# NilFoundation/crypto3-zk

Hardware: AMD Instinct MI355X
Metric: MSM Mpoints/sec, BLS12-381 G1 Pippenger, 2^20 points per GPU (higher is better)
Workload: dtype u32; 1 GPU; BLS12-381 G1 Pippenger MSM, ONE MSM of 1 x 2^20 random points/scalars, bases resident; points_per_gpu=1048576, parallelism=point-range partition x1 + one all-gather of the 144-B partial sums

## Files before the change

__graft_entry__.py:

```python
import importlib.util
import os
import subprocess
import sys

ROOT = os.path.dirname(os.path.abspath(__file__))


def _load_pkg():
    if "crypto3_zk_amd" in sys.modules:
        return sys.modules["crypto3_zk_amd"]
    pkg_dir = os.path.join(ROOT, "crypto3-zk_amd")
    spec = importlib.util.spec_from_file_location("crypto3_zk_amd", os.path.join(pkg_dir, "__init__.py"),
                                                  submodule_search_locations=[pkg_dir])
    mod = importlib.util.module_from_spec(spec)
    sys.modules["crypto3_zk_amd"] = mod
    spec.loader.exec_module(mod)
    return mod


def build() -> None:
    env = dict(os.environ)
    subprocess.check_call(["make", "-C", os.path.join(ROOT, "crypto3-zk_amd"), "-j4", "all"], env=env)
    subprocess.check_call(["make", "-C", os.path.join(ROOT, "oracle"), "liboracle.so"], env=env)
    subprocess.check_call(["make", "-j2", "-C", os.path.join(ROOT, "tests", "cpp")], env=env)
    subprocess.check_call(["make", "-C", os.path.join(ROOT, "tests", "cpp"), "-f", "merkle.mk"], env=env)
    subprocess.check_call(["make", "-C", os.path.join(ROOT, "tests", "cpp"), "-f", "pow.mk"], env=env)
    subprocess.check_call(["make", "-j2", "-C", os.path.join(ROOT, "tests", "cpp"), "-f", "pasta.mk"], env=env)
    subprocess.check_call(["make", "-C", os.path.join(ROOT, "tests", "cpp"), "-f", "wide.mk"], env=env)
    subprocess.check_call(["make", "-C", os.path.join(ROOT, "tests", "cpp"), "-f", "entries.mk"], env=env)
    subprocess.check_call(["make", "-C", os.path.join(ROOT, "tests", "cpp"), "-f", "ipa.mk"], env=env)
    subprocess.check_call(["make", "-C", os.path.join(ROOT, "tests", "cpp"), "-f", "lagrange.mk"], env=env)
    subprocess.check_call(["make", "-C", os.path.join(ROOT, "tests", "cpp"), "-f", "ceremony.mk"], env=env)
    subprocess.check_call(["make", "-C", os.path.join(ROOT, "tests", "cpp"), "-f", "fri_query.mk"], env=env)
    subprocess.check_call(["make", "-C", os.path.join(ROOT, "tests", "cpp"), "-f", "ipp2.mk"], env=env)
    zk = _load_pkg()
    zk.load_library()


def smoke() -> None:
    import numpy as np

    sys.path.insert(0, os.path.join(ROOT, "oracle"))
    import cport as cp
    import pyoracle as po

    zk = _load_pkg()
    ctx = zk.Context(0)
    n = 5000
    ks = cp.random_fr(0, 1, n)
    bases = ctx.bases_from_scalars(zk.BLS12_381, zk.G1, ks)
    pts, inf = bases.download()
    exp_pts, _ = cp.batch_mul(0, 1, ks)
    assert (pts == exp_pts).all(), "device fixed-base multiples differ from the oracle"
    sc = cp.random_fr(0, 2, n)
    aff, is_inf = ctx.msm_affine(bases, sc)
    exp, einf = cp.msm(0, 1, pts, sc, chunks=2)
    assert is_inf == einf and (aff == exp).all(), "MSM differs from the oracle"
    grp = zk.DeviceGroup([0, 0])
    gb = grp.upload_bases(zk.BLS12_381, zk.G1, pts)
    gaff, ginf = grp.msm_affine(gb, sc)
    assert ginf == einf and (gaff == exp).all(), "device-group MSM differs from the oracle"
    gb.free()
    grp.close()
    k2 = cp.random_fr(0, 4, 300)
    b2 = ctx.bases_from_scalars(zk.BLS12_381, zk.G2, k2)
    p2, _ = b2.download()
    s2 = cp.random_fr(0, 5, 300)
    aff2, inf2 = ctx.msm_affine(b2, s2)
    exp2, einf2 = cp.msm(0, 2, p2, s2, chunks=2)
    assert inf2 == einf2 and (aff2 == exp2).all(), "G2 MSM differs from the oracle"
    b2.free()
    log_m = 12
    w = np.array(po.to_limbs(po.BLS12_381.root_of_unity(log_m), 4), dtype=np.uint64)
    a = cp.random_fr(0, 3, 2 << log_m).reshape(2, 1 << log_m, 4)
    got = ctx.ntt(zk.BLS12_381, a, log_m, w)
    assert (got == cp.ntt(0, a, log_m, w)).all(), "NTT differs from the oracle"
    assert (ctx.ntt(zk.BLS12_381, got, log_m, w, inverse=True) == a).all()
    bases.free()
    M, nin = 1024, 10
    g16 = cp.Groth16(0, M, nin, seed=3)
    kind, m = cp.domain_choice(M + nin + 1, 32)
    wd = np.array(po.to_limbs(po.BLS12_381.root_of_unity((M + nin).bit_length()), 4), dtype=np.uint64)
    gen = np.array(po.to_limbs(po.BLS12_381.fr_generator, 4), dtype=np.uint64)
    g16.set_domain(kind, m, wd)
    r1cs = ctx.upload_r1cs(zk.BLS12_381, g16.M, g16.n, g16.N, g16.csr(0), g16.csr(1), g16.csr(2))
    assert (r1cs.kind, r1cs.m) == (kind, m) == (2, 1040), "the constraint system's domain is not the reference's choice"
    z = np.concatenate([np.array([[1, 0, 0, 0]], dtype=np.uint64), g16.assignment()])
    assert (ctx.groth16_witness_h(r1cs, z, wd, gen) == g16.witness_map(wd, gen)).all(), "witness map over the step domain differs from the oracle"
    r1cs.free()
    import hashlib
    state = hashlib.sha256(b"zkhip smoke").digest()
    k = next(k for k in range(1 << 20)
             if int.from_bytes(hashlib.sha256(hashlib.sha256(state + (12345 + k).to_bytes(4, "big")).digest()).digest()[28:], "big") & 0xFFF == 0)
    assert ctx.pow_grind(state, 12345, 0xFFF) == (12345 + k, k + 1), "the device's proof of work is not the first accepted nonce"
    ctx.close()
    print("smoke ok: G1 MSM n=5000 (one context and a device group of two), G2 MSM n=300, NTT 2^12 x 2 and the witness map over a step radix-2 domain bit-exact against the oracle; proof of work (12 bits) = the reference loop's nonce")


if __name__ == "__main__":
    build()
    if len(sys.argv) > 1 and sys.argv[1] == "smoke":
        smoke()
```

crypto3-zk_amd/csrc/msm_entries.hip:

```cpp
#include <algorithm>
#include <string>

#include "ctx.hpp"
#include "fu.hpp"
#include "msm_entries.hpp"
#include "msm_ops.hpp"
#include "msm_recode.hpp"

namespace {

using namespace zkhip;

constexpr uint32_t MSM_LARGE_BUCKET = 128;
constexpr uint32_t MSM_LARGE_CHUNK = 4096;

template <uint32_t THREADS>
ZK_D void block_inclusive_scan(uint32_t *scratch) {
    const uint32_t t = threadIdx.x;
    __syncthreads();
    for (uint32_t d = 1; d < THREADS; d <<= 1) {
        uint32_t x = t >= d ? scratch[t - d] : 0;
        __syncthreads();
        scratch[t] += x;
        __syncthreads();
    }
}

__global__ __launch_bounds__(256) void msm_scan_local(const uint32_t *__restrict__ hist, uint32_t count, uint32_t *__restrict__ offs,
                                                      uint32_t *__restrict__ block_sums) {
    __shared__ uint32_t part[256];
    const uint32_t t = threadIdx.x, base = blockIdx.x * 1024 + t * 4;
    uint32_t v[4], s = 0;
#pragma unroll
    for (int k = 0; k < 4; ++k) {
        v[k] = base + k < count ? hist[base + k] : 0;
        s += v[k];
    }
    part[t] = s;
    block_inclusive_scan<256>(part);
    uint32_t run = part[t] - s;
#pragma unroll
    for (int k = 0; k < 4; ++k) {
        if (base + k < count) offs[base + k] = run;
        run += v[k];
    }
    if (t == 255) block_sums[blockIdx.x] = part[255];
}

__global__ __launch_bounds__(1024) void msm_scan_top(uint32_t *__restrict__ block_sums, uint32_t nblocks, uint32_t *__restrict__ total) {
    __shared__ uint32_t part[1024];
    const uint32_t t = threadIdx.x;
    const uint32_t per = (nblocks + 1023) / 1024;
    const uint32_t lo = min(nblocks, t * per), hi = min(nblocks, lo + per);
    uint32_t s = 0;
    for (uint32_t i = lo; i < hi; ++i) s += block_sums[i];
    part[t] = s;
    block_inclusive_scan<1024>(part);
    uint32_t run = part[t] - s;
    for (uint32_t i = lo; i < hi; ++i) {
        uint32_t x = block_sums[i];
        block_sums[i] = run;
        run += x;
    }
    if (t == 1023) *total = part[1023];
}

__global__ __launch_bounds__(256) void msm_scan_add(uint32_t *__restrict__ offs, uint32_t count, const uint32_t *__restrict__ block_sums,
                                                    uint32_t *__restrict__ cursor) {
    const uint32_t base = blockIdx.x * 1024 + threadIdx.x * 4;
    const uint32_t add = block_sums[blockIdx.x];
#pragma unroll
    for (int k = 0; k < 4; ++k) {
        if (base + k < count) {
            uint32_t x = offs[base + k] + add;
            offs[base + k] = x;
            cursor[base + k] = x;
        }
    }
}

__global__ __launch_bounds__(1024) void msm_scan_single(const uint32_t *__restrict__ hist, uint32_t count, uint32_t *__restrict__ offs,
                                                        uint32_t *__restrict__ cursor) {
    __shared__ uint32_t part[1024];
    __shared__ uint32_t carry;
    const uint32_t t = threadIdx.x;
    if (t == 0) carry = 0;
    __syncthreads();
    for (uint32_t base = 0; base < count; base += 1024) {
        const uint32_t v = base + t < count ? hist[base + t] : 0;
        part[t] = v;
        block_inclusive_scan<1024>(part);
        const uint32_t excl = carry + part[t] - v;
        if (base + t < count) {
            offs[base + t] = excl;
            if (cursor != offs) cursor[base + t] = excl;
        }
        __syncthreads();
        if (t == 1023) carry += part[1023];
        __syncthreads();
    }
    if (t == 0) offs[count] = carry;
}
constexpr uint32_t MSM_SCAN_SINGLE_MAX = 1u << 16;

inline int msm_scan(zkhip_ctx *ctx, const char *name, const uint32_t *hist, uint32_t count, uint32_t *offs, uint32_t *bsums) {
    if (count <= MSM_SCAN_SINGLE_MAX) {
        ZK_LAUNCH(ctx, name, msm_scan_single, dim3(1), dim3(1024), 0, hist, count, offs, offs);
        return 0;
    }
    const uint32_t nblk = (count + 1023) / 1024;
    ZK_LAUNCH(ctx, name, msm_scan_local, dim3(nblk), dim3(256), 0, hist, count, offs, bsums);
    ZK_LAUNCH(ctx, name, msm_scan_top, dim3(1), dim3(1024), 0, bsums, nblk, offs + count);
    ZK_LAUNCH(ctx, name, msm_scan_add, dim3(nblk), dim3(256), 0, offs, count, bsums, offs);
    return 0;
}

template <class FR>
__global__ __launch_bounds__(256) void msm_digits_only(const uint32_t *__restrict__ scalars, uint32_t n, MsmWindows win, uint32_t wrank,
                                                       uint32_t wworld, uint32_t *__restrict__ dig) {
    uint32_t i = blockIdx.x * blockDim.x + threadIdx.x;
    if (i >= n) return;
    uint32_t s[8];
    const uint32_t flip = msm_fold_scalar<FR>(scalars + (size_t)i * 8, s) ? 0x80000000u : 0u;
    uint32_t carry = 0, next = wrank, lw = 0;
    for (int w = 0; w < win.W; ++w) {
        uint32_t d = msm_recode(s, win.off(w), win.width(w), carry);
        if ((uint32_t)w != next) continue;
        dig[(size_t)lw * n + i] = d == DIG_NONE ? d : d ^ flip;
        next += wworld;
        ++lw;
    }
}

struct SortBig {
    static constexpr uint32_t TILE = 16384, THREADS = 1024;
};
struct SortSmall {
    static constexpr uint32_t TILE = 4096, THREADS = 256;
};
constexpr uint32_t SORT_MAX_LOW = 10;
constexpr uint32_t SORT_MAX_SUPER = 1024;

ZK_D uint32_t sort_key(const SortGeom &g, uint32_t w, uint32_t d) { return (w % g.S) * g.B + (d & 0x7FFFFFFFu); }
ZK_D uint32_t sort_entry(const SortGeom &g, uint32_t w, uint32_t i, uint32_t d) {
    return ((g.tables ? (g.slot0 + w) * g.bases_n : 0u) + g.base_off + i) | (d & 0x80000000u);
}

template <class SZ>
__global__ __launch_bounds__(SZ::THREADS) void msm_sort_hist(const uint32_t *__restrict__ dig, SortGeom g, uint32_t *__restrict__ bh) {
    constexpr uint32_t SORT_TILE = SZ::TILE, SORT_THREADS = SZ::THREADS;
    extern __shared__ uint32_t lh[];
    const uint32_t tile = blockIdx.x, w = blockIdx.y, t = threadIdx.x;
    for (uint32_t k = t; k < g.nsuper; k += SORT_THREADS) lh[k] = 0;
    __syncthreads();
    const uint32_t lo = tile * SORT_TILE, hi = min(g.n, lo + SORT_TILE);
    for (uint32_t i = lo + t; i < hi; i += SORT_THREADS) {
        uint32_t d = dig[(size_t)w * g.n + i];
        if (d != DIG_NONE) atomicAdd(&lh[sort_key(g, w, d) >> g.lowb], 1u);
    }
    __syncthreads();
    const size_t col = (size_t)w * g.ntile + tile, stride = (size_t)g.W * g.ntile;
    for (uint32_t k = t; k < g.nsuper; k += SORT_THREADS) bh[(size_t)k * stride + col] = lh[k];
}

template <uint32_t SORT_THREADS>
ZK_D uint32_t block_excl_scan(uint32_t *v, uint32_t count, uint32_t *scratch ) {
    const uint32_t t = threadIdx.x, per = (count + SORT_THREADS - 1) / SORT_THREADS;
    const uint32_t lo = min(count, t * per), hi = min(count, lo + per);
    uint32_t s = 0;
    for (uint32_t k = lo; k < hi; ++k) s += v[k];
    scratch[t] = s;
    block_inclusive_scan<SORT_THREADS>(scratch);
    const uint32_t total = scratch[SORT_THREADS - 1];
    uint32_t run = scratch[t] - s;
    for (uint32_t k = lo; k < hi; ++k) {
        uint32_t x = v[k];
        v[k] = run;
        run += x;
    }
    __syncthreads();
    return total;
}

template <class SZ>
__global__ __launch_bounds__(SZ::THREADS) void msm_sort_split(const uint32_t *__restrict__ dig, SortGeom g, const uint32_t *__restrict__ bo,
                                                              uint32_t *__restrict__ tmp_idx, uint16_t *__restrict__ tmp_key) {
    constexpr uint32_t SORT_TILE = SZ::TILE, SORT_THREADS = SZ::THREADS;
    extern __shared__ uint32_t sm[];
    uint32_t *loff = sm;
    uint32_t *cur = loff + g.nsuper + 1;
    uint32_t *gbase = cur + g.nsuper;
    uint32_t *scratch = gbase + g.nsuper;
    uint32_t *sidx = scratch + SORT_THREADS;
    uint32_t *skey = sidx + SORT_TILE;
    const uint32_t tile = blockIdx.x, w = blockIdx.y, t = threadIdx.x;
    const size_t col = (size_t)w * g.ntile + tile, stride = (size_t)g.W * g.ntile;
    for (uint32_t k = t; k < g.nsuper; k += SORT_THREADS) {
        loff[k] = 0;
        gbase[k] = bo[(size_t)k * stride + col];
    }
    __syncthreads();
    const uint32_t lo = tile * SORT_TILE, hi = min(g.n, lo + SORT_TILE);
    for (uint32_t i = lo + t; i < hi; i += SORT_THREADS) {
        uint32_t d = dig[(size_t)w * g.n + i];
        if (d != DIG_NONE) atomicAdd(&loff[sort_key(g, w, d) >> g.lowb], 1u);
    }
    __syncthreads();
    const uint32_t total = block_excl_scan<SORT_THREADS>(loff, g.nsuper, scratch);
    if (t == 0) loff[g.nsuper] = total;
    for (uint32_t k = t; k < g.nsuper; k += SORT_THREADS) cur[k] = loff[k];
    __syncthreads();
    for (uint32_t i = lo + t; i < hi; i += SORT_THREADS) {
        uint32_t d = dig[(size_t)w * g.n + i];
        if (d == DIG_NONE) continue;
        const uint32_t key = sort_key(g, w, d);
        const uint32_t r = atomicAdd(&cur[key >> g.lowb], 1u);
        sidx[r] = sort_entry(g, w, i, d);
        skey[r] = key;
    }
    __syncthreads();
    const uint32_t lmask = (1u << g.lowb) - 1;
    for (uint32_t s = t; s < total; s += SORT_THREADS) {
        const uint32_t key = skey[s], bin = key >> g.lowb, pos = gbase[bin] + (s - loff[bin]);
        tmp_idx[pos] = sidx[s];
        tmp_key[pos] = (uint16_t)(key & lmask);
    }
}

constexpr uint32_t SORT_NLOW_MAX = 1u << SORT_MAX_LOW;

template <uint32_t THREADS>
ZK_D void block_scan_counts(const uint32_t *cnt, uint32_t *excl, uint32_t *scratch) {
    constexpr uint32_t CPT = SORT_NLOW_MAX / THREADS;
    const uint32_t t = threadIdx.x;
    uint32_t s = 0;
#pragma unroll
    for (uint32_t k = 0; k < CPT; ++k) s += cnt[t * CPT + k];
    scratch[t] = s;
    block_inclusive_scan<THREADS>(scratch);
    uint32_t run = scratch[t] - s;
#pragma unroll
    for (uint32_t k = 0; k < CPT; ++k) {
        excl[t * CPT + k] = run;
        run += cnt[t * CPT + k];
    }
    __syncthreads();
}

template <class SZ>
__global__ __launch_bounds__(SZ::THREADS) void msm_sort_final(const uint32_t *__restrict__ tmp_idx, const uint16_t *__restrict__ tmp_key, SortGeom g,
                                                              uint32_t nb, const uint32_t *__restrict__ bo, uint32_t *__restrict__ offs,
                                                              uint32_t *__restrict__ idx) {
    constexpr uint32_t SORT_TILE = SZ::TILE, SORT_THREADS = SZ::THREADS;
    __shared__ uint32_t cnt[SORT_NLOW_MAX], cursor[SORT_NLOW_MAX], loff[SORT_NLOW_MAX], cur[SORT_NLOW_MAX], scratch[SORT_THREADS];
    extern __shared__ uint32_t sm[];
    uint32_t *sidx = sm;
    uint16_t *skey = reinterpret_cast<uint16_t *>(sidx + SORT_TILE);
    const uint32_t grp = blockIdx.x, t = threadIdx.x;
    const size_t stride = (size_t)g.W * g.ntile;
    const uint32_t start = bo[(size_t)grp * stride];
    const uint32_t end = bo[(size_t)(grp + 1) * stride];
    const uint32_t nlow = 1u << g.lowb;
    for (uint32_t k = t; k < SORT_NLOW_MAX; k += SORT_THREADS) cnt[k] = 0;
    __syncthreads();
    for (uint32_t k = start + t; k < end; k += SORT_THREADS) atomicAdd(&cnt[tmp_key[k]], 1u);
    __syncthreads();
    block_scan_counts<SORT_THREADS>(cnt, cursor, scratch);
    for (uint32_t k = t; k < nlow; k += SORT_THREADS) {
        const uint32_t bucket = grp * nlow + k;
        cursor[k] += start;
        if (bucket < nb) offs[bucket] = cursor[k];
    }
    if (grp + 1 == g.nsuper && t == 0) offs[nb] = end;
    __syncthreads();
    for (uint32_t c0 = start; c0 < end; c0 += SORT_TILE) {
        const uint32_t c1 = min(end, c0 + SORT_TILE);
        for (uint32_t k = t; k < SORT_NLOW_MAX; k += SORT_THREADS) cnt[k] = 0;
        __syncthreads();
        for (uint32_t k = c0 + t; k < c1; k += SORT_THREADS) atomicAdd(&cnt[tmp_key[k]], 1u);
        __syncthreads();
        block_scan_counts<SORT_THREADS>(cnt, loff, scratch);
        for (uint32_t k = t; k < SORT_NLOW_MAX; k += SORT_THREADS) cur[k] = loff[k];
        __syncthreads();
        for (uint32_t k = c0 + t; k < c1; k += SORT_THREADS) {
            const uint32_t key = tmp_key[k];
            const uint32_t r = atomicAdd(&cur[key], 1u);
            sidx[r] = tmp_idx[k];
            skey[r] = (uint16_t)key;
        }
        __syncthreads();
        for (uint32_t s = t; s < c1 - c0; s += SORT_THREADS) {
            const uint32_t key = skey[s];
            idx[cursor[key] + (s - loff[key])] = sidx[s];
        }
        __syncthreads();
        for (uint32_t k = t; k < SORT_NLOW_MAX; k += SORT_THREADS) cursor[k] += cnt[k];
        __syncthreads();
    }
}

constexpr uint32_t SIZE_BINS = MSM_LARGE_BUCKET + 2;

ZK_HD uint32_t size_bin(uint32_t size, uint32_t large) {
    if (size == 0 || size > large) return SIZE_BINS - 1;
    return size > MSM_LARGE_BUCKET ? 0 : 1 + MSM_LARGE_BUCKET - size;
}

__global__ __launch_bounds__(256) void msm_size_hist(const uint32_t *__restrict__ offs, uint32_t nbuckets, uint32_t nblocks,
                                                     uint32_t large, uint32_t *__restrict__ bh) {
    __shared__ uint32_t lh[SIZE_BINS];
    const uint32_t t = threadIdx.x;
    if (t < SIZE_BINS) lh[t] = 0;
    __syncthreads();
    for (uint32_t g = blockIdx.x * 1024 + t; g < min(nbuckets, (blockIdx.x + 1) * 1024); g += 256)
        atomicAdd(&lh[size_bin(offs[g + 1] - offs[g], large)], 1u);
    __syncthreads();
    if (t < SIZE_BINS) bh[(size_t)t * nblocks + blockIdx.x] = lh[t];
}

__global__ __launch_bounds__(256) void msm_size_scatter(const uint32_t *__restrict__ offs, uint32_t nbuckets, uint32_t nblocks,
                                                        uint32_t large, const uint32_t *__restrict__ bo, uint32_t *__restrict__ order) {
    __shared__ uint32_t cur[SIZE_BINS];
    const uint32_t t = threadIdx.x;
    if (t < SIZE_BINS) cur[t] = bo[(size_t)t * nblocks + blockIdx.x];
    __syncthreads();
    for (uint32_t g = blockIdx.x * 1024 + t; g < min(nbuckets, (blockIdx.x + 1) * 1024); g += 256)
        order[atomicAdd(&cur[size_bin(offs[g + 1] - offs[g], large)], 1u)] = g;
}

__global__ __launch_bounds__(256) void msm_plan_large(const uint32_t *__restrict__ offs, uint32_t nbuckets, uint32_t *__restrict__ plan,
                                                      uint32_t *__restrict__ tasks, uint32_t *__restrict__ large, uint32_t task_cap,
                                                      uint32_t large_cap, uint32_t thresh, uint32_t *__restrict__ status) {
    uint32_t g = blockIdx.x * blockDim.x + threadIdx.x;
    if (g >= nbuckets) return;
    uint32_t lo = offs[g], hi = offs[g + 1], size = hi - lo;
    if (size <= thresh) return;
    uint32_t nt = (size + MSM_LARGE_CHUNK - 1) / MSM_LARGE_CHUNK;
    uint32_t first = atomicAdd(&plan[0], nt);
    uint32_t slot = atomicAdd(&plan[1], 1u);
    if (first + nt > task_cap || slot >= large_cap) {
        atomicOr(status, ZK_STATUS_MSM_PLAN_OVERFLOW);
        return;
    }
    for (uint32_t t = 0; t < nt; ++t) {
        tasks[3 * (first + t)] = g;
        tasks[3 * (first + t) + 1] = lo + t * MSM_LARGE_CHUNK;
        tasks[3 * (first + t) + 2] = min(hi, lo + (t + 1) * MSM_LARGE_CHUNK);
    }
    large[3 * slot] = g;
    large[3 * slot + 1] = first;
    large[3 * slot + 2] = nt;
}

inline MsmPlan msm_plan(const zkhip_ctx *ctx, const zkhip_bases *bases, size_t n) {
    MsmPlan p;
    p.tables = bases->tables();
    int c = p.tables ? bases->c_tab : ctx->opt_msm_window_bits;
    if (c <= 0) c = zk_msm_auto_window(n);
    p.c = std::max(2, std::min(ZK_MSM_MAX_C, c));
    if (!p.tables) p.c = std::min(p.c, 16);
    p.W_all = msm_windows(zk_scalar_bits(bases->curve), p.c);
    p.win = msm_make_windows(zk_scalar_bits(bases->curve), p.W_all);
    p.wrank = p.tables ? (uint32_t)bases->win_rank : 0u;
    p.wworld = p.tables ? (uint32_t)bases->win_world : 1u;
    p.W = p.tables ? bases->local_windows() : p.W_all;
    p.B = 1u << (p.c - 1);
    if (!p.tables) p.S = (uint32_t)p.W;
    else {
        int s = ctx->opt_msm_sets;
        if (s <= 0) s = (int)((zk_msm_target_lanes() + p.B - 1) / p.B);
        p.S = (uint32_t)std::max(1, std::min(p.W, s));
        while (p.S > 1 && (uint64_t)p.S * p.B > ((uint64_t)SORT_MAX_SUPER << SORT_MAX_LOW)) --p.S;
    }
    p.nb = p.S * p.B;
    return p;
}

template <class SZ>
int msm_sort_run(zkhip_ctx *ctx, const SortGeom &g, uint32_t nbh, const uint32_t *dig, uint32_t *bh, uint32_t *bo, uint32_t *bsums, uint32_t *tmp_idx,
                 uint16_t *tmp_key, uint32_t *offs, uint32_t *idx) {
    const size_t lds_hist = (size_t)g.nsuper * 4;
    const size_t lds_split = ((size_t)3 * g.nsuper + 1 + SZ::THREADS + 2 * SZ::TILE) * 4;
    const size_t lds_final = (size_t)SZ::TILE * 6;
    if (lds_split > 48 * 1024) ZK_MAX_LDS(ctx, msm_sort_split<SZ>, 160 * 1024 - 256);
    if (lds_final > 40 * 1024) ZK_MAX_LDS(ctx, msm_sort_final<SZ>, 160 * 1024 - (4 * SORT_NLOW_MAX + SZ::THREADS) * 4 - 256);
    ZK_LAUNCH(ctx, "msm_sort_hist", msm_sort_hist<SZ>, dim3(g.ntile, g.W), dim3(SZ::THREADS), lds_hist, dig, g, bh);
    ZK_TRY(msm_scan(ctx, "msm_scan", bh, nbh, bo, bsums));
    ZK_LAUNCH(ctx, "msm_sort_split", msm_sort_split<SZ>, dim3(g.ntile, g.W), dim3(SZ::THREADS), lds_split, dig, g, bo, tmp_idx, tmp_key);
    ZK_LAUNCH(ctx, "msm_sort_final", msm_sort_final<SZ>, dim3(g.nsuper), dim3(SZ::THREADS), lds_final, tmp_idx, tmp_key, g, g.S * g.B, bo, offs, idx);
    return 0;
}

}

int zk_msm_entries_plan(const zkhip_ctx *ctx, const zkhip_bases *bases, size_t offset, size_t n, MsmEntriesCall &c, std::string &error) {
    const MsmPlan &P = c.P = msm_plan(ctx, bases, n);
    if ((uint64_t)P.W * n >= (1ull << 32) || (uint64_t)bases->nslots * bases->n >= (1ull << 31)) {
        error = "MSM of " + std::to_string(n) + " points x " + std::to_string(P.W) + " windows exceeds the 32-bit entry index (split the range)";
        return ZKHIP_ERR_RANGE;
    }
    SortGeom &g = c.g;
    g.n = (uint32_t)n;
    g.W = (uint32_t)P.W;
    g.B = P.B;
    g.S = P.S;
    g.lowb = (uint32_t)std::min<int>(SORT_MAX_LOW, P.c - 1);
    g.nsuper = (P.nb + (1u << g.lowb) - 1) >> g.lowb;
    c.big_tiles = ctx->opt_msm_sort_tile_log >= 14;
    g.tile = c.big_tiles ? SortBig::TILE : SortSmall::TILE;
    g.ntile = (uint32_t)((n + g.tile - 1) / g.tile);
    g.tables = P.tables ? 1u : 0u;
    g.slot0 = P.tables ? (uint32_t)bases->slot_of_local(0) : 0u;
    g.bases_n = (uint32_t)bases->n;
    g.base_off = (uint32_t)offset;
    if (g.nsuper > SORT_MAX_SUPER) return ZKHIP_ERR_RANGE;
    const size_t nbh64 = (size_t)g.nsuper * g.W * g.ntile;
    if (nbh64 >= (1ull << 31)) return ZKHIP_ERR_RANGE;
    c.nbh = (uint32_t)nbh64;
    c.sblk = (P.nb + 1023) / 1024;
    c.nsh = SIZE_BINS * c.sblk;
    c.large_thresh = (uint32_t)std::max<size_t>(MSM_LARGE_BUCKET, 4 * ((c.entries() + P.nb - 1) / P.nb));
    c.large_cap = (uint32_t)(c.entries() / c.large_thresh + 1);
    c.task_cap = (uint32_t)(c.entries() / MSM_LARGE_CHUNK + c.large_cap + 1);
    return 0;
}

int zk_msm_entries(zkhip_ctx *ctx, int curve, const MsmEntriesCall &c, const MsmEntriesBuffers &w, const uint32_t *d_scalars) {
    const MsmPlan &P = c.P;
    const uint32_t n = c.g.n, nb = P.nb;
    ZK_TRY(fr_sat_dispatch(curve, [&](auto fr) -> int {
        typedef typename decltype(fr)::type FR;
        ZK_LAUNCH(ctx, "msm_digits", msm_digits_only<FR>, grid_1d(n), dim3(256), 0, d_scalars, n, P.win, P.wrank, P.wworld, w.dig);
        return 0;
    }));
    ZK_TRY((c.big_tiles ? msm_sort_run<SortBig> : msm_sort_run<SortSmall>)(ctx, c.g, c.nbh, w.dig, w.bh, w.bo, w.bsums, w.tmp_idx, w.tmp_key, w.offs, w.idx));
    ZK_LAUNCH(ctx, "msm_size_sort", msm_size_hist, dim3(c.sblk), dim3(256), 0, w.offs, nb, c.sblk, c.large_thresh, w.sh);
    ZK_TRY(msm_scan(ctx, "msm_size_sort", w.sh, c.nsh, w.so, w.ssums));
    ZK_LAUNCH(ctx, "msm_size_sort", msm_size_scatter, dim3(c.sblk), dim3(256), 0, w.offs, nb, c.sblk, c.large_thresh, w.so, w.order);
    return 0;
}

int zk_msm_large_plan(zkhip_ctx *ctx, const MsmEntriesCall &c, const MsmEntriesBuffers &w) {
    const uint32_t nb = c.P.nb;
    ZK_HIP_CHECK(ctx, hipMemsetAsync(w.plan, 0, 16, ctx->stream));
    ZK_LAUNCH(ctx, "msm_plan_large", msm_plan_large, grid_1d(nb), dim3(256), 0, w.offs, nb, w.plan, w.tasks, w.large, c.task_cap, c.large_cap,
              c.large_thresh, ctx->d_status);
    return 0;
}

uint32_t zk_msm_size_bin(uint32_t size, uint32_t large) { return size_bin(size, large); }
```

crypto3-zk_amd/csrc/msm_entries.hpp:

```cpp
#pragma once
#include <string>

#include "ctx.hpp"
#include "msm_recode.hpp"

namespace zkhip {

struct MsmPlan {
    int c, W_all, W;
    uint32_t B, S, nb;
    MsmWindows win;
    uint32_t wrank, wworld;
    bool tables;
};

struct SortGeom {
    uint32_t n;
    uint32_t W;
    uint32_t B;
    uint32_t S;
    uint32_t lowb;
    uint32_t nsuper;
    uint32_t tile;
    uint32_t ntile;
    uint32_t slot0;
    uint32_t tables;
    uint32_t bases_n;
    uint32_t base_off;
};

struct MsmEntriesCall {
    MsmPlan P;
    SortGeom g;
    bool big_tiles;
    uint32_t nbh;
    uint32_t sblk, nsh;
    uint32_t large_thresh, large_cap, task_cap;
    size_t entries() const { return (size_t)P.W * g.n; }
};

struct MsmEntriesBuffers {
    uint32_t *dig, *bh, *bo, *bsums, *tmp_idx;
    uint16_t *tmp_key;
    uint32_t *offs, *idx;
    uint32_t *sh, *so, *ssums, *order;
    uint32_t *plan, *tasks, *large;
};

}

int zk_msm_entries_plan(const zkhip_ctx *ctx, const zkhip_bases *bases, size_t offset, size_t n, zkhip::MsmEntriesCall &c, std::string &error);
int zk_msm_entries(zkhip_ctx *ctx, int curve, const zkhip::MsmEntriesCall &c, const zkhip::MsmEntriesBuffers &w, const uint32_t *d_scalars);
int zk_msm_large_plan(zkhip_ctx *ctx, const zkhip::MsmEntriesCall &c, const zkhip::MsmEntriesBuffers &w);
uint32_t zk_msm_size_bin(uint32_t size, uint32_t large);
```

Baseline: 399.5 Mpoints/s.

## Cut kernel launches and barriers across MSM bucket sort and size-sort pipeline

Replaces the barrier-heavy LDS block scan with a wave-shuffle scan and merges the scan-top and scan-add kernels into a single kernel that sums the preceding block totals. The size histogram is folded into the sort-final kernel when there are 1024 low buckets. Large-bucket planning moves into the size-scatter kernel, and plan zeroing moves into the digits kernel, removing one kernel and a memset. The split and final sort kernels now keep their tile in registers, and the scatter pass uses per-wave segments so output order is deterministic. This trims launch overhead and memory passes in the MSM preprocessing. The cost is more complex code, more register pressure and higher correctness risk.

Result: faster. 421.9 Mpoints/s, median of 6 (+5.6%).

```diff
diff --git a/__graft_entry__.py b/__graft_entry__.py
--- a/__graft_entry__.py
+++ b/__graft_entry__.py
@@ -28,6 +28,7 @@
     subprocess.check_call(["make", "-j2", "-C", os.path.join(ROOT, "tests", "cpp"), "-f", "pasta.mk"], env=env)
     subprocess.check_call(["make", "-C", os.path.join(ROOT, "tests", "cpp"), "-f", "wide.mk"], env=env)
     subprocess.check_call(["make", "-C", os.path.join(ROOT, "tests", "cpp"), "-f", "entries.mk"], env=env)
+    subprocess.check_call(["make", "-j2", "-C", os.path.join(ROOT, "tests", "cpp"), "-f", "entries_latency.mk"], env=env)
     subprocess.check_call(["make", "-C", os.path.join(ROOT, "tests", "cpp"), "-f", "ipa.mk"], env=env)
     subprocess.check_call(["make", "-C", os.path.join(ROOT, "tests", "cpp"), "-f", "lagrange.mk"], env=env)
     subprocess.check_call(["make", "-C", os.path.join(ROOT, "tests", "cpp"), "-f", "ceremony.mk"], env=env)
diff --git a/crypto3-zk_amd/csrc/msm_block_scan.hpp b/crypto3-zk_amd/csrc/msm_block_scan.hpp
--- /dev/null
+++ b/crypto3-zk_amd/csrc/msm_block_scan.hpp
@@ -0,0 +1,37 @@
+#pragma once
+#include <cstdint>
+
+#include "zk_defs.hpp"
+
+#if defined(__HIPCC__)
+namespace zkhip {
+
+ZK_D uint32_t wave_sum(uint32_t x) {
+#pragma unroll
+    for (int d = 32; d > 0; d >>= 1) x += __shfl_xor(x, d, 64);
+    return x;
+}
+
+template <uint32_t THREADS>
+ZK_D void block_inclusive_scan(uint32_t *scratch) {
+    constexpr uint32_t WAVES = THREADS / 64;
+    static_assert(THREADS % 64 == 0 && WAVES <= 16, "one LDS word per wave total, at most 16 of them");
+    __shared__ uint32_t wave_total[WAVES];
+    const uint32_t t = threadIdx.x, lane = t & 63, wave = t >> 6;
+    uint32_t x = scratch[t];
+#pragma unroll
+    for (int d = 1; d < 64; d <<= 1) {
+        const uint32_t y = __shfl_up(x, d, 64);
+        if (lane >= (uint32_t)d) x += y;
+    }
+    if (lane == 63) wave_total[wave] = x;
+    __syncthreads();
+    uint32_t below = 0;
+#pragma unroll
+    for (uint32_t k = 0; k + 1 < WAVES; ++k) below += k < wave ? wave_total[k] : 0u;
+    scratch[t] = x + below;
+    __syncthreads();
+}
+
+}
+#endif
diff --git a/crypto3-zk_amd/csrc/msm_entries.hip b/crypto3-zk_amd/csrc/msm_entries.hip
--- a/crypto3-zk_amd/csrc/msm_entries.hip
+++ b/crypto3-zk_amd/csrc/msm_entries.hip
@@ -3,6 +3,7 @@
 
 #include "ctx.hpp"
 #include "fu.hpp"
+#include "msm_block_scan.hpp"
 #include "msm_entries.hpp"
 #include "msm_ops.hpp"
 #include "msm_recode.hpp"
@@ -13,18 +14,6 @@
 
 constexpr uint32_t MSM_LARGE_BUCKET = 128;
 constexpr uint32_t MSM_LARGE_CHUNK = 4096;
-
-template <uint32_t THREADS>
-ZK_D void block_inclusive_scan(uint32_t *scratch) {
-    const uint32_t t = threadIdx.x;
-    __syncthreads();
-    for (uint32_t d = 1; d < THREADS; d <<= 1) {
-        uint32_t x = t >= d ? scratch[t - d] : 0;
-        __syncthreads();
-        scratch[t] += x;
-        __syncthreads();
-    }
-}
 
 __global__ __launch_bounds__(256) void msm_scan_local(const uint32_t *__restrict__ hist, uint32_t count, uint32_t *__restrict__ offs,
                                                       uint32_t *__restrict__ block_sums) {
@@ -47,56 +36,31 @@
     if (t == 255) block_sums[blockIdx.x] = part[255];
 }
 
-__global__ __launch_bounds__(1024) void msm_scan_top(uint32_t *__restrict__ block_sums, uint32_t nblocks, uint32_t *__restrict__ total) {
+__global__ __launch_bounds__(256) void msm_scan_add(uint32_t *__restrict__ offs, uint32_t count, const uint32_t *__restrict__ block_sums) {
+    __shared__ uint32_t wave_total[4];
+    const uint32_t t = threadIdx.x, blk = blockIdx.x, base = blk * 1024 + t * 4;
+    uint32_t s = 0;
+    for (uint32_t i = t; i < blk; i += 256) s += block_sums[i];
+    s = wave_sum(s);
+    if ((t & 63) == 0) wave_total[t >> 6] = s;
+    __syncthreads();
+    const uint32_t add = wave_total[0] + wave_total[1] + wave_total[2] + wave_total[3];
+#pragma unroll
+    for (int k = 0; k < 4; ++k)
+        if (base + k < count) offs[base + k] += add;
+    if (blk + 1 == gridDim.x && t == 0) offs[count] = add + block_sums[blk];
+}
+
+__global__ __launch_bounds__(1024) void msm_scan_single(const uint32_t *__restrict__ hist, uint32_t count, uint32_t *__restrict__ offs) {
     __shared__ uint32_t part[1024];
     const uint32_t t = threadIdx.x;
-    const uint32_t per = (nblocks + 1023) / 1024;
-    const uint32_t lo = min(nblocks, t * per), hi = min(nblocks, lo + per);
-    uint32_t s = 0;
-    for (uint32_t i = lo; i < hi; ++i) s += block_sums[i];
-    part[t] = s;
-    block_inclusive_scan<1024>(part);
-    uint32_t run = part[t] - s;
-    for (uint32_t i = lo; i < hi; ++i) {
-        uint32_t x = block_sums[i];
-        block_sums[i] = run;
-        run += x;
-    }
-    if (t == 1023) *total = part[1023];
-}
-
-__global__ __launch_bounds__(256) void msm_scan_add(uint32_t *__restrict__ offs, uint32_t count, const uint32_t *__restrict__ block_sums,
-                                                    uint32_t *__restrict__ cursor) {
-    const uint32_t base = blockIdx.x * 1024 + threadIdx.x * 4;
-    const uint32_t add = block_sums[blockIdx.x];
-#pragma unroll
-    for (int k = 0; k < 4; ++k) {
-        if (base + k < count) {
-            uint32_t x = offs[base + k] + add;
-            offs[base + k] = x;
-            cursor[base + k] = x;
-        }
-    }
-}
-
-__global__ __launch_bounds__(1024) void msm_scan_single(const uint32_t *__restrict__ hist, uint32_t count, uint32_t *__restrict__ offs,
-                                                        uint32_t *__restrict__ cursor) {
-    __shared__ uint32_t part[1024];
-    __shared__ uint32_t carry;
-    const uint32_t t = threadIdx.x;
-    if (t == 0) carry = 0;
-    __syncthreads();
+    uint32_t carry = 0;
     for (uint32_t base = 0; base < count; base += 1024) {
         const uint32_t v = base + t < count ? hist[base + t] : 0;
         part[t] = v;
         block_inclusive_scan<1024>(part);
-        const uint32_t excl = carry + part[t] - v;
-        if (base + t < count) {
-            offs[base + t] = excl;
-            if (cursor != offs) cursor[base + t] = excl;
-        }
-        __syncthreads();
-        if (t == 1023) carry += part[1023];
+        if (base + t < count) offs[base + t] = carry + part[t] - v;
+        carry += part[1023];
         __syncthreads();
     }
     if (t == 0) offs[count] = carry;
@@ -105,21 +69,21 @@
 
 inline int msm_scan(zkhip_ctx *ctx, const char *name, const uint32_t *hist, uint32_t count, uint32_t *offs, uint32_t *bsums) {
     if (count <= MSM_SCAN_SINGLE_MAX) {
-        ZK_LAUNCH(ctx, name, msm_scan_single, dim3(1), dim3(1024), 0, hist, count, offs, offs);
+        ZK_LAUNCH(ctx, name, msm_scan_single, dim3(1), dim3(1024), 0, hist, count, offs);
         return 0;
     }
     const uint32_t nblk = (count + 1023) / 1024;
     ZK_LAUNCH(ctx, name, msm_scan_local, dim3(nblk), dim3(256), 0, hist, count, offs, bsums);
-    ZK_LAUNCH(ctx, name, msm_scan_top, dim3(1), dim3(1024), 0, bsums, nblk, offs + count);
-    ZK_LAUNCH(ctx, name, msm_scan_add, dim3(nblk), dim3(256), 0, offs, count, bsums, offs);
+    ZK_LAUNCH(ctx, name, msm_scan_add, dim3(nblk), dim3(256), 0, offs, count, bsums);
     return 0;
 }
 
 template <class FR>
 __global__ __launch_bounds__(256) void msm_digits_only(const uint32_t *__restrict__ scalars, uint32_t n, MsmWindows win, uint32_t wrank,
-                                                       uint32_t wworld, uint32_t *__restrict__ dig) {
+                                                       uint32_t wworld, uint32_t *__restrict__ dig, uint32_t *__restrict__ plan) {
     uint32_t i = blockIdx.x * blockDim.x + threadIdx.x;
     if (i >= n) return;
+    if (i == 0) plan[0] = plan[1] = 0;
     uint32_t s[8];
     const uint32_t flip = msm_fold_scalar<FR>(scalars + (size_t)i * 8, s) ? 0x80000000u : 0u;
     uint32_t carry = 0, next = wrank, lw = 0;
@@ -134,6 +98,9 @@
 
 struct SortBig {
     static constexpr uint32_t TILE = 16384, THREADS = 1024;
+};
+struct SortMid {
+    static constexpr uint32_t TILE = 8192, THREADS = 512;
 };
 struct SortSmall {
     static constexpr uint32_t TILE = 4096, THREADS = 256;
@@ -185,7 +152,7 @@
 template <class SZ>
 __global__ __launch_bounds__(SZ::THREADS) void msm_sort_split(const uint32_t *__restrict__ dig, SortGeom g, const uint32_t *__restrict__ bo,
                                                               uint32_t *__restrict__ tmp_idx, uint16_t *__restrict__ tmp_key) {
-    constexpr uint32_t SORT_TILE = SZ::TILE, SORT_THREADS = SZ::THREADS;
+    constexpr uint32_t SORT_TILE = SZ::TILE, SORT_THREADS = SZ::THREADS, ITEMS = SORT_TILE / SORT_THREADS;
     extern __shared__ uint32_t sm[];
     uint32_t *loff = sm;
     uint32_t *cur = loff + g.nsuper + 1;
@@ -195,27 +162,32 @@
     uint32_t *skey = sidx + SORT_TILE;
     const uint32_t tile = blockIdx.x, w = blockIdx.y, t = threadIdx.x;
     const size_t col = (size_t)w * g.ntile + tile, stride = (size_t)g.W * g.ntile;
+    const uint32_t lo = tile * SORT_TILE, hi = min(g.n, lo + SORT_TILE);
+    uint32_t d[ITEMS];
+#pragma unroll
+    for (uint32_t j = 0; j < ITEMS; ++j) {
+        const uint32_t i = lo + j * SORT_THREADS + t;
+        d[j] = i < hi ? dig[(size_t)w * g.n + i] : DIG_NONE;
+    }
     for (uint32_t k = t; k < g.nsuper; k += SORT_THREADS) {
         loff[k] = 0;
         gbase[k] = bo[(size_t)k * stride + col];
     }
     __syncthreads();
-    const uint32_t lo = tile * SORT_TILE, hi = min(g.n, lo + SORT_TILE);
-    for (uint32_t i = lo + t; i < hi; i += SORT_THREADS) {
-        uint32_t d = dig[(size_t)w * g.n + i];
-        if (d != DIG_NONE) atomicAdd(&loff[sort_key(g, w, d) >> g.lowb], 1u);
-    }
+#pragma unroll
+    for (uint32_t j = 0; j < ITEMS; ++j)
+        if (d[j] != DIG_NONE) atomicAdd(&loff[sort_key(g, w, d[j]) >> g.lowb], 1u);
     __syncthreads();
     const uint32_t total = block_excl_scan<SORT_THREADS>(loff, g.nsuper, scratch);
     if (t == 0) loff[g.nsuper] = total;
     for (uint32_t k = t; k < g.nsuper; k += SORT_THREADS) cur[k] = loff[k];
     __syncthreads();
-    for (uint32_t i = lo + t; i < hi; i += SORT_THREADS) {
-        uint32_t d = dig[(size_t)w * g.n + i];
-        if (d == DIG_NONE) continue;
-        const uint32_t key = sort_key(g, w, d);
+#pragma unroll
+    for (uint32_t j = 0; j < ITEMS; ++j) {
+        if (d[j] == DIG_NONE) continue;
+        const uint32_t key = sort_key(g, w, d[j]);
         const uint32_t r = atomicAdd(&cur[key >> g.lowb], 1u);
-        sidx[r] = sort_entry(g, w, i, d);
+        sidx[r] = sort_entry(g, w, lo + j * SORT_THREADS + t, d[j]);
         skey[r] = key;
     }
     __syncthreads();
@@ -247,12 +219,43 @@
     __syncthreads();
 }
 
+constexpr uint32_t SIZE_BINS = MSM_LARGE_BUCKET + 2;
+
+ZK_HD uint32_t size_bin(uint32_t size, uint32_t large) {
+    if (size == 0 || size > large) return SIZE_BINS - 1;
+    return size > MSM_LARGE_BUCKET ? 0 : 1 + MSM_LARGE_BUCKET - size;
+}
+
+template <uint32_t THREADS>
+ZK_D void block_scan_chunk(uint32_t *cnt, uint32_t *cursor, uint32_t *cur, uint32_t *dst, uint32_t *scratch) {
+    constexpr uint32_t CPT = SORT_NLOW_MAX / THREADS;
+    const uint32_t t = threadIdx.x;
+    uint32_t s = 0;
+#pragma unroll
+    for (uint32_t k = 0; k < CPT; ++k) s += cnt[t * CPT + k];
+    scratch[t] = s;
+    block_inclusive_scan<THREADS>(scratch);
+    uint32_t run = scratch[t] - s;
+#pragma unroll
+    for (uint32_t k = 0; k < CPT; ++k) {
+        const uint32_t i = t * CPT + k, c = cnt[i];
+        cur[i] = run;
+        dst[i] = cursor[i] - run;
+        cursor[i] += c;
+        cnt[i] = 0;
+        run += c;
+    }
+    __syncthreads();
+}
+
 template <class SZ>
 __global__ __launch_bounds__(SZ::THREADS) void msm_sort_final(const uint32_t *__restrict__ tmp_idx, const uint16_t *__restrict__ tmp_key, SortGeom g,
                                                               uint32_t nb, const uint32_t *__restrict__ bo, uint32_t *__restrict__ offs,
-                                                              uint32_t *__restrict__ idx) {
-    constexpr uint32_t SORT_TILE = SZ::TILE, SORT_THREADS = SZ::THREADS;
-    __shared__ uint32_t cnt[SORT_NLOW_MAX], cursor[SORT_NLOW_MAX], loff[SORT_NLOW_MAX], cur[SORT_NLOW_MAX], scratch[SORT_THREADS];
+                                                              uint32_t *__restrict__ idx, uint32_t large, uint32_t *__restrict__ sh) {
+    constexpr uint32_t SORT_TILE = SZ::TILE, SORT_THREADS = SZ::THREADS, ITEMS = SORT_TILE / SORT_THREADS;
+    constexpr uint32_t NO_KEY = 0xFFFFu;
+    static_assert(SORT_THREADS >= SIZE_BINS, "one lane per size bin");
+    __shared__ uint32_t cnt[SORT_NLOW_MAX], cursor[SORT_NLOW_MAX], dst[SORT_NLOW_MAX], cur[SORT_NLOW_MAX], scratch[SORT_THREADS];
     extern __shared__ uint32_t sm[];
     uint32_t *sidx = sm;
     uint16_t *skey = reinterpret_cast<uint16_t *>(sidx + SORT_TILE);
@@ -262,48 +265,47 @@
     const uint32_t end = bo[(size_t)(grp + 1) * stride];
     const uint32_t nlow = 1u << g.lowb;
     for (uint32_t k = t; k < SORT_NLOW_MAX; k += SORT_THREADS) cnt[k] = 0;
+    if (t < SIZE_BINS) cur[t] = 0;
     __syncthreads();
     for (uint32_t k = start + t; k < end; k += SORT_THREADS) atomicAdd(&cnt[tmp_key[k]], 1u);
     __syncthreads();
     block_scan_counts<SORT_THREADS>(cnt, cursor, scratch);
-    for (uint32_t k = t; k < nlow; k += SORT_THREADS) {
+    for (uint32_t k = t; k < SORT_NLOW_MAX; k += SORT_THREADS) {
         const uint32_t bucket = grp * nlow + k;
         cursor[k] += start;
-        if (bucket < nb) offs[bucket] = cursor[k];
+        if (k < nlow && bucket < nb) {
+            offs[bucket] = cursor[k];
+            if (sh) atomicAdd(&cur[size_bin(cnt[k], large)], 1u);
+        }
+        cnt[k] = 0;
     }
     if (grp + 1 == g.nsuper && t == 0) offs[nb] = end;
     __syncthreads();
+    if (sh && t < SIZE_BINS) sh[(size_t)t * g.nsuper + grp] = cur[t];
     for (uint32_t c0 = start; c0 < end; c0 += SORT_TILE) {
         const uint32_t c1 = min(end, c0 + SORT_TILE);
-        for (uint32_t k = t; k < SORT_NLOW_MAX; k += SORT_THREADS) cnt[k] = 0;
+        uint32_t key[ITEMS], entry[ITEMS];
+#pragma unroll
+        for (uint32_t j = 0; j < ITEMS; ++j) {
+            const uint32_t k = c0 + j * SORT_THREADS + t;
+            key[j] = k < c1 ? tmp_key[k] : NO_KEY;
+            entry[j] = k < c1 ? tmp_idx[k] : 0u;
+        }
+#pragma unroll
+        for (uint32_t j = 0; j < ITEMS; ++j)
+            if (key[j] != NO_KEY) atomicAdd(&cnt[key[j]], 1u);
         __syncthreads();
-        for (uint32_t k = c0 + t; k < c1; k += SORT_THREADS) atomicAdd(&cnt[tmp_key[k]], 1u);
-        __syncthreads();
-        block_scan_counts<SORT_THREADS>(cnt, loff, scratch);
-        for (uint32_t k = t; k < SORT_NLOW_MAX; k += SORT_THREADS) cur[k] = loff[k];
-        __syncthreads();
-        for (uint32_t k = c0 + t; k < c1; k += SORT_THREADS) {
-            const uint32_t key = tmp_key[k];
-            const uint32_t r = atomicAdd(&cur[key], 1u);
-            sidx[r] = tmp_idx[k];
-            skey[r] = (uint16_t)key;
+        block_scan_chunk<SORT_THREADS>(cnt, cursor, cur, dst, scratch);
+#pragma unroll
+        for (uint32_t j = 0; j < ITEMS; ++j) {
+            if (key[j] == NO_KEY) continue;
+            const uint32_t r = atomicAdd(&cur[key[j]], 1u);
+            sidx[r] = entry[j];
+            skey[r] = (uint16_t)key[j];
         }
         __syncthreads();
-        for (uint32_t s = t; s < c1 - c0; s += SORT_THREADS) {
-            const uint32_t key = skey[s];
-            idx[cursor[key] + (s - loff[key])] = sidx[s];
-        }
-        __syncthreads();
-        for (uint32_t k = t; k < SORT_NLOW_MAX; k += SORT_THREADS) cursor[k] += cnt[k];
-        __syncthreads();
-    }
-}
-
-constexpr uint32_t SIZE_BINS = MSM_LARGE_BUCKET + 2;
-
-ZK_HD uint32_t size_bin(uint32_t size, uint32_t large) {
-    if (size == 0 || size > large) return SIZE_BINS - 1;
-    return size > MSM_LARGE_BUCKET ? 0 : 1 + MSM_LARGE_BUCKET - size;
+        for (uint32_t s = t; s < c1 - c0; s += SORT_THREADS) idx[dst[skey[s]] + s] = sidx[s];
+    }
 }
 
 __global__ __launch_bounds__(256) void msm_size_hist(const uint32_t *__restrict__ offs, uint32_t nbuckets, uint32_t nblocks,
@@ -318,38 +320,62 @@
     if (t < SIZE_BINS) bh[(size_t)t * nblocks + blockIdx.x] = lh[t];
 }
 
+struct LargePlan {
+    uint32_t *plan, *tasks, *large;
+    uint32_t task_cap, large_cap;
+    uint32_t *status;
+};
+
+ZK_D void msm_plan_bucket(const LargePlan &p, uint32_t g, uint32_t lo, uint32_t hi) {
+    const uint32_t nt = (hi - lo + MSM_LARGE_CHUNK - 1) / MSM_LARGE_CHUNK;
+    const uint32_t first = atomicAdd(&p.plan[0], nt);
+    const uint32_t slot = atomicAdd(&p.plan[1], 1u);
+    if (first + nt > p.task_cap || slot >= p.large_cap) {
+        atomicOr(p.status, ZK_STATUS_MSM_PLAN_OVERFLOW);
+        return;
+    }
+    for (uint32_t t = 0; t < nt; ++t) {
+        p.tasks[3 * (first + t)] = g;
+        p.tasks[3 * (first + t) + 1] = lo + t * MSM_LARGE_CHUNK;
+        p.tasks[3 * (first + t) + 2] = min(hi, lo + (t + 1) * MSM_LARGE_CHUNK);
+    }
+    p.large[3 * slot] = g;
+    p.large[3 * slot + 1] = first;
+    p.large[3 * slot + 2] = nt;
+}
+
 __global__ __launch_bounds__(256) void msm_size_scatter(const uint32_t *__restrict__ offs, uint32_t nbuckets, uint32_t nblocks,
-                                                        uint32_t large, const uint32_t *__restrict__ bo, uint32_t *__restrict__ order) {
-    __shared__ uint32_t cur[SIZE_BINS];
-    const uint32_t t = threadIdx.x;
-    if (t < SIZE_BINS) cur[t] = bo[(size_t)t * nblocks + blockIdx.x];
-    __syncthreads();
-    for (uint32_t g = blockIdx.x * 1024 + t; g < min(nbuckets, (blockIdx.x + 1) * 1024); g += 256)
-        order[atomicAdd(&cur[size_bin(offs[g + 1] - offs[g], large)], 1u)] = g;
-}
-
-__global__ __launch_bounds__(256) void msm_plan_large(const uint32_t *__restrict__ offs, uint32_t nbuckets, uint32_t *__restrict__ plan,
-                                                      uint32_t *__restrict__ tasks, uint32_t *__restrict__ large, uint32_t task_cap,
-                                                      uint32_t large_cap, uint32_t thresh, uint32_t *__restrict__ status) {
-    uint32_t g = blockIdx.x * blockDim.x + threadIdx.x;
-    if (g >= nbuckets) return;
-    uint32_t lo = offs[g], hi = offs[g + 1], size = hi - lo;
-    if (size <= thresh) return;
-    uint32_t nt = (size + MSM_LARGE_CHUNK - 1) / MSM_LARGE_CHUNK;
-    uint32_t first = atomicAdd(&plan[0], nt);
-    uint32_t slot = atomicAdd(&plan[1], 1u);
-    if (first + nt > task_cap || slot >= large_cap) {
-        atomicOr(status, ZK_STATUS_MSM_PLAN_OVERFLOW);
-        return;
-    }
-    for (uint32_t t = 0; t < nt; ++t) {
-        tasks[3 * (first + t)] = g;
-        tasks[3 * (first + t) + 1] = lo + t * MSM_LARGE_CHUNK;
-        tasks[3 * (first + t) + 2] = min(hi, lo + (t + 1) * MSM_LARGE_CHUNK);
-    }
-    large[3 * slot] = g;
-    large[3 * slot + 1] = first;
-    large[3 * slot + 2] = nt;
+                                                        uint32_t large, const uint32_t *__restrict__ bo, uint32_t *__restrict__ order, LargePlan plan) {
+    constexpr uint32_t SEGS = 16;
+    __shared__ uint32_t seg[SEGS * SIZE_BINS];
+    const uint32_t t = threadIdx.x, first = blockIdx.x * 1024, last = min(nbuckets, first + 1024);
+    for (uint32_t k = t; k < SEGS * SIZE_BINS; k += 256) seg[k] = 0;
+    __syncthreads();
+    uint32_t slot[4], rank[4];
+#pragma unroll
+    for (uint32_t j = 0; j < 4; ++j) {
+        const uint32_t g = first + j * 256 + t;
+        if (g >= last) continue;
+        const uint32_t lo = offs[g], hi = offs[g + 1];
+        slot[j] = (j * 4 + (t >> 6)) * SIZE_BINS + size_bin(hi - lo, large);
+        rank[j] = atomicAdd(&seg[slot[j]], 1u);
+        if (hi - lo > large) msm_plan_bucket(plan, g, lo, hi);
+    }
+    __syncthreads();
+    if (t < SIZE_BINS) {
+        uint32_t run = bo[(size_t)t * nblocks + blockIdx.x];
+        for (uint32_t s = 0; s < SEGS; ++s) {
+            const uint32_t x = seg[s * SIZE_BINS + t];
+            seg[s * SIZE_BINS + t] = run;
+            run += x;
+        }
+    }
+    __syncthreads();
+#pragma unroll
+    for (uint32_t j = 0; j < 4; ++j) {
+        const uint32_t g = first + j * 256 + t;
+        if (g < last) order[seg[slot[j]] + rank[j]] = g;
+    }
 }
 
 inline MsmPlan msm_plan(const zkhip_ctx *ctx, const zkhip_bases *bases, size_t n) {
@@ -377,17 +403,17 @@
 }
 
 template <class SZ>
-int msm_sort_run(zkhip_ctx *ctx, const SortGeom &g, uint32_t nbh, const uint32_t *dig, uint32_t *bh, uint32_t *bo, uint32_t *bsums, uint32_t *tmp_idx,
-                 uint16_t *tmp_key, uint32_t *offs, uint32_t *idx) {
+int msm_sort_run(zkhip_ctx *ctx, const SortGeom &g, uint32_t nbh, const MsmEntriesBuffers &w, uint32_t large, uint32_t *sh) {
     const size_t lds_hist = (size_t)g.nsuper * 4;
     const size_t lds_split = ((size_t)3 * g.nsuper + 1 + SZ::THREADS + 2 * SZ::TILE) * 4;
     const size_t lds_final = (size_t)SZ::TILE * 6;
     if (lds_split > 48 * 1024) ZK_MAX_LDS(ctx, msm_sort_split<SZ>, 160 * 1024 - 256);
     if (lds_final > 40 * 1024) ZK_MAX_LDS(ctx, msm_sort_final<SZ>, 160 * 1024 - (4 * SORT_NLOW_MAX + SZ::THREADS) * 4 - 256);
-    ZK_LAUNCH(ctx, "msm_sort_hist", msm_sort_hist<SZ>, dim3(g.ntile, g.W), dim3(SZ::THREADS), lds_hist, dig, g, bh);
-    ZK_TRY(msm_scan(ctx, "msm_scan", bh, nbh, bo, bsums));
-    ZK_LAUNCH(ctx, "msm_sort_split", msm_sort_split<SZ>, dim3(g.ntile, g.W), dim3(SZ::THREADS), lds_split, dig, g, bo, tmp_idx, tmp_key);
-    ZK_LAUNCH(ctx, "msm_sort_final", msm_sort_final<SZ>, dim3(g.nsuper), dim3(SZ::THREADS), lds_final, tmp_idx, tmp_key, g, g.S * g.B, bo, offs, idx);
+    ZK_LAUNCH(ctx, "msm_sort_hist", msm_sort_hist<SZ>, dim3(g.ntile, g.W), dim3(SZ::THREADS), lds_hist, w.dig, g, w.bh);
+    ZK_TRY(msm_scan(ctx, "msm_scan", w.bh, nbh, w.bo, w.bsums));
+    ZK_LAUNCH(ctx, "msm_sort_split", msm_sort_split<SZ>, dim3(g.ntile, g.W), dim3(SZ::THREADS), lds_split, w.dig, g, w.bo, w.tmp_idx, w.tmp_key);
+    ZK_LAUNCH(ctx, "msm_sort_final", msm_sort_final<SZ>, dim3(g.nsuper), dim3(SZ::THREADS), lds_final, w.tmp_idx, w.tmp_key, g, g.S * g.B, w.bo, w.offs, w.idx,
+              large, sh);
     return 0;
 }
 
@@ -406,8 +432,8 @@
     g.S = P.S;
     g.lowb = (uint32_t)std::min<int>(SORT_MAX_LOW, P.c - 1);
     g.nsuper = (P.nb + (1u << g.lowb) - 1) >> g.lowb;
-    c.big_tiles = ctx->opt_msm_sort_tile_log >= 14;
-    g.tile = c.big_tiles ? SortBig::TILE : SortSmall::TILE;
+    const int tile_log = ctx->opt_msm_sort_tile_log;
+    g.tile = tile_log >= 14 ? SortBig::TILE : tile_log == 13 ? SortMid::TILE : SortSmall::TILE;
     g.ntile = (uint32_t)((n + g.tile - 1) / g.tile);
     g.tables = P.tables ? 1u : 0u;
     g.slot0 = P.tables ? (uint32_t)bases->slot_of_local(0) : 0u;
@@ -430,22 +456,21 @@
     const uint32_t n = c.g.n, nb = P.nb;
     ZK_TRY(fr_sat_dispatch(curve, [&](auto fr) -> int {
         typedef typename decltype(fr)::type FR;
-        ZK_LAUNCH(ctx, "msm_digits", msm_digits_only<FR>, grid_1d(n), dim3(256), 0, d_scalars, n, P.win, P.wrank, P.wworld, w.dig);
+        ZK_LAUNCH(ctx, "msm_digits", msm_digits_only<FR>, grid_1d(n), dim3(256), 0, d_scalars, n, P.win, P.wrank, P.wworld, w.dig, w.plan);
         return 0;
     }));
-    ZK_TRY((c.big_tiles ? msm_sort_run<SortBig> : msm_sort_run<SortSmall>)(ctx, c.g, c.nbh, w.dig, w.bh, w.bo, w.bsums, w.tmp_idx, w.tmp_key, w.offs, w.idx));
-    ZK_LAUNCH(ctx, "msm_size_sort", msm_size_hist, dim3(c.sblk), dim3(256), 0, w.offs, nb, c.sblk, c.large_thresh, w.sh);
+    const bool final_counts_sizes = (1u << c.g.lowb) == 1024;
+    uint32_t *sh = final_counts_sizes ? w.sh : nullptr;
+    ZK_TRY((c.g.tile == SortBig::TILE   ? msm_sort_run<SortBig>
+            : c.g.tile == SortMid::TILE ? msm_sort_run<SortMid>
+                                        : msm_sort_run<SortSmall>)(ctx, c.g, c.nbh, w, c.large_thresh, sh));
+    if (!final_counts_sizes) ZK_LAUNCH(ctx, "msm_size_sort", msm_size_hist, dim3(c.sblk), dim3(256), 0, w.offs, nb, c.sblk, c.large_thresh, w.sh);
     ZK_TRY(msm_scan(ctx, "msm_size_sort", w.sh, c.nsh, w.so, w.ssums));
-    ZK_LAUNCH(ctx, "msm_size_sort", msm_size_scatter, dim3(c.sblk), dim3(256), 0, w.offs, nb, c.sblk, c.large_thresh, w.so, w.order);
+    const LargePlan plan = {w.plan, w.tasks, w.large, c.task_cap, c.large_cap, ctx->d_status};
+    ZK_LAUNCH(ctx, "msm_plan_large", msm_size_scatter, dim3(c.sblk), dim3(256), 0, w.offs, nb, c.sblk, c.large_thresh, w.so, w.order, plan);
     return 0;
 }
 
-int zk_msm_large_plan(zkhip_ctx *ctx, const MsmEntriesCall &c, const MsmEntriesBuffers &w) {
-    const uint32_t nb = c.P.nb;
-    ZK_HIP_CHECK(ctx, hipMemsetAsync(w.plan, 0, 16, ctx->stream));
-    ZK_LAUNCH(ctx, "msm_plan_large", msm_plan_large, grid_1d(nb), dim3(256), 0, w.offs, nb, w.plan, w.tasks, w.large, c.task_cap, c.large_cap,
-              c.large_thresh, ctx->d_status);
-    return 0;
-}
+int zk_msm_large_plan(zkhip_ctx *, const MsmEntriesCall &, const MsmEntriesBuffers &) { return 0; }
 
 uint32_t zk_msm_size_bin(uint32_t size, uint32_t large) { return size_bin(size, large); }
diff --git a/crypto3-zk_amd/csrc/msm_entries.hpp b/crypto3-zk_amd/csrc/msm_entries.hpp
--- a/crypto3-zk_amd/csrc/msm_entries.hpp
+++ b/crypto3-zk_amd/csrc/msm_entries.hpp
@@ -32,7 +32,6 @@
 struct MsmEntriesCall {
     MsmPlan P;
     SortGeom g;
-    bool big_tiles;
     uint32_t nbh;
     uint32_t sblk, nsh;
     uint32_t large_thresh, large_cap, task_cap;
```
